# sd196821/QuadSim

Measured on AMD Instinct MI355X. Metric: env-steps/sec at N parallel envs (1/2/4/8 GPU); per-step state L2 err vs NumPy ref, higher is better.
Workload: dtype f32

## Files before the change

### quadsim_amd/csrc/private_queue.hpp

```cpp
#pragma once

struct QsChainLane {
    hsa_queue_t *queue = nullptr;
    char *kernargs = nullptr;
    std::vector<uint64_t> slot_qidx;
    uint64_t issued = 0;
    int64_t tile0 = 0, tile_end = 0;
    hsa_signal_t done{};
    void *rev_ptr = nullptr;
    hsa_signal_t rev{};
    int64_t rev_value = 0;
    char *res_kernarg = nullptr;
    hsa_signal_t res_done{};
    bool res_launched = false;
    uint64_t res_prog = 0;
};

struct QsKernel {
    uint64_t object = 0;
    uint32_t kernarg_size = 0, group_size = 0, private_size = 0;
    unsigned block = 0;
};

struct QsChain {
// ... 7 lines not shown
    std::vector<char> image;
    uint64_t kernel_object = 0;
    int v_integ = -1, v_params = -1, v_rmode = -1, v_split = -1, v_prep = -1;
    uint32_t kernarg_size = 0, group_size = 0, private_size = 0;
    unsigned block = 0;
    size_t stride = 0, slots = 0;
    unsigned *d_owner = nullptr;
    unsigned *d_err = nullptr;
    volatile unsigned *h_err = nullptr;
    bool kernargs_on_device = false;
    bool dirty = false;
    bool hip_dirty = true;
    bool stream_ordered = false;
    void *fwd_ptr = nullptr;
    hsa_signal_t fwd{};
    uint64_t fwd_seq = 0;
    int dbg_shift = 0;
    bool pkt_unreleased = false;
    bool res_enabled = false;
    bool res_dbg_packets = false;
    bool res_open = false;
    bool res_fits = false;
    QsKernel res_kernel;
    int rv_integ = -1, rv_params = -1, rv_rmode = -1, rv_prep = -1;
    int64_t res_wave_cap = 0;
    unsigned long long *ring = nullptr;
    size_t ring_slots = 0;
    uint64_t res_issued = 1;
    uint64_t res_retired = 1;
    uint64_t res_seq0 = 0;
    uint64_t res_idle_ticks = 0;
    uint64_t res_dispatches = 0;
    unsigned long long *d_rseq = nullptr;
    unsigned *d_rcnt = nullptr;
    volatile unsigned long long *h_res = nullptr;
    unsigned long long *d_hres = nullptr;
};

namespace {

#define HSA_TRY(expr)                                                                                   \
    do {                                                                                                \
        hsa_status_t s_ = (expr);                                                                       \
        if (s_ != HSA_STATUS_SUCCESS) {                                                                 \
            const char *m_ = nullptr;                                                                   \
            hsa_status_string(s_, &m_);                                                                 \
            return fail(QS_ERR_HIP, "%s failed: %s", #expr, m_ ? m_ : "unknown HSA status");           \
        }                                                                                               \
// ... 107 lines not shown
}

void chain_close(QsEnv *e)
{
    QsChain *c = e->chain;
    if (!c) return;
    if (c->fwd.handle) hsa_signal_store_screlease(c->fwd, INT64_MAX);
    for (QsChainLane &L : c->lanes) {
        if (L.queue) hsa_queue_destroy(L.queue);
        if (L.kernargs) hsa_amd_memory_pool_free(L.kernargs);
        if (L.done.handle) hsa_signal_destroy(L.done);
        if (L.rev_ptr) (void)hipFree(L.rev_ptr);
        if (L.res_kernarg) hsa_amd_memory_pool_free(L.res_kernarg);
        if (L.res_done.handle) hsa_signal_destroy(L.res_done);
    }
    if (c->ring) hsa_amd_memory_pool_free(c->ring);
    if (c->d_rseq) (void)hipFree(c->d_rseq);
    if (c->d_rcnt) (void)hipFree(c->d_rcnt);
    if (c->h_res) (void)hipHostFree((void *)c->h_res);
    if (c->fwd_ptr) (void)hipFree(c->fwd_ptr);
    if (c->have_exe) hsa_executable_destroy(c->exe);
    if (c->have_reader) hsa_code_object_reader_destroy(c->reader);
    if (c->d_owner) (void)hipFree(c->d_owner);
    if (c->h_err) (void)hipHostFree((void *)c->h_err);
    delete c;
    e->chain = nullptr;
}

int chain_resolve_kernel(QsEnv *e)
{
    QsChain *c = e->chain;
    const int integ = e->cfg.integrator == QS_INTEG_FROZEN ? 0 : 1;
    const int rmode = e->init ? 3 : e->cfg.randomise;
    const int params = (rmode == 2 || e->per_env_params) ? 1 : 0;
    static const int forced = getenv("QS_SPLIT") ? atoi(getenv("QS_SPLIT")) : -1;
    const int split = (forced >= 0 ? forced != 0 : e->n <= kSplitMaxEnvs) ? 1 : 0;
    int64_t lane_tiles = 0;
    for (const QsChainLane &L : c->lanes) lane_tiles = std::max<int64_t>(lane_tiles, L.tile_end - L.tile0);
    if (c->lanes.empty()) lane_tiles = e->tiles;
    const int prep = split ? prep_for(rmode, lane_tiles) : 0;
    if (c->kernel_object && integ == c->v_integ && rmode == c->v_rmode && params == c->v_params && split == c->v_split && prep == c->v_prep) return QS_OK;
    char sym[160];
    if (split) snprintf(sym, sizeof sym, "_ZN12_GLOBAL__N_111k_env_splitILi%dELb%dELi%dELi%dEEEvNS_8StepArgsE.kd", integ, params, rmode, prep);
    else snprintf(sym, sizeof sym, "_ZN12_GLOBAL__N_15k_envILi%dELb%dELi%dEEEvNS_8StepArgsE.kd", integ, params, rmode);
    hsa_executable_symbol_t ks;
    uint64_t ko = 0;
// ... 28 lines not shown
{
    int can = 0;
    return hipDeviceGetAttribute(&can, hipDeviceAttributeCanUseStreamWaitValue, e->cfg.device) == hipSuccess && can != 0;
}

int chain_enable_stream_order(QsEnv *e)
{
    QsChain *c = e->chain;
    if (!c->fwd_ptr) {
        int r = chain_alloc_hip_signal(&c->fwd_ptr, &c->fwd, 0);
        if (r) return r;
        c->fwd_seq = 0;
    }
    for (QsChainLane &L : c->lanes) {
        if (L.rev_ptr) continue;
        int r = chain_alloc_hip_signal(&L.rev_ptr, &L.rev, kRevStart);
        if (r) return r;
        L.rev_value = kRevStart;
    }
    c->stream_ordered = true;
    return QS_OK;
}

int chain_open(QsEnv *e, int nq)
{
    if (e->cfg.kind == QS_KIND_HOVERING_V0) return fail(QS_ERR_INVALID, "qs_set_queue_mode: docking envs only");
    if (e->cfg.io_space != QS_IO_DEVICE) return fail(QS_ERR_INVALID, "qs_set_queue_mode: device buffers only");
    QsChain *c = new (std::nothrow) QsChain();
    if (!c) return fail(QS_ERR_NOMEM, "qs_set_queue_mode: out of host memory");
    e->chain = c;
    auto body = [&]() -> int {
        HSA_TRY(hsa_init());
        char bus[32] = "";
        AgentPick pick{0xffffffffu, 0, e->cfg.device, 0, {}, {}, false, false};
        unsigned dom = 0, b = 0, d = 0, f = 0;
        if (hipDeviceGetPCIBusId(bus, sizeof bus, e->cfg.device) == hipSuccess && sscanf(bus, "%x:%x:%x.%x", &dom, &b, &d, &f) == 4) {
            pick.want_bdf = (b << 8) | (d << 3) | f;
            pick.want_domain = dom;
        }
        HSA_TRY(hsa_iterate_agents(chain_agent_cb, &pick));
        if (!pick.have_gpu || !pick.have_cpu) return fail(QS_ERR_HIP, "qs_set_queue_mode: no HSA agent for device %d (%s)", e->cfg.device, bus);
        c->gpu = pick.gpu; c->cpu = pick.cpu;
        hsa_status_t ps = hsa_amd_agent_iterate_memory_pools(c->cpu, chain_kernarg_pool_cb, &c->kernarg_pool);
        if (ps != HSA_STATUS_INFO_BREAK) return fail(QS_ERR_HIP, "qs_set_queue_mode: no kernarg memory pool");
        int r = chain_read_code_object(c->image);
        if (r) return r;
// ... 23 lines not shown
            L.tile0 = cut[q]; L.tile_end = cut[q + 1];
            HSA_TRY(hsa_queue_create(c->gpu, 4096, HSA_QUEUE_TYPE_SINGLE, nullptr, nullptr, UINT32_MAX, UINT32_MAX, &L.queue));
            if (dp.found) {
                HSA_TRY(hsa_amd_memory_pool_allocate(dp.pool, c->stride * c->slots, 0, (void **)&L.kernargs));
                HSA_TRY(hsa_amd_agents_allow_access(1, &c->cpu, nullptr, L.kernargs));
            } else {
                HSA_TRY(hsa_amd_memory_pool_allocate(c->kernarg_pool, c->stride * c->slots, 0, (void **)&L.kernargs));
                HSA_TRY(hsa_amd_agents_allow_access(1, &c->gpu, nullptr, L.kernargs));
            }
            memset(L.kernargs, 0, c->stride * c->slots);
            L.slot_qidx.assign(c->slots, 0);
            HSA_TRY(hsa_signal_create(0, 0, nullptr, &L.done));
        }
        HIP_TRY(hipMalloc((void **)&c->d_owner, (size_t)e->tiles * sizeof(unsigned)));
        HIP_TRY(hipHostMalloc((void **)&c->h_err, 64, hipHostMallocMapped | hipHostMallocCoherent));
        *c->h_err = 0;
        HIP_TRY(hipHostGetDevicePointer((void **)&c->d_err, (void *)c->h_err, 0));
        const char *res = getenv("QS_RESIDENT");
        c->res_enabled = dp.found && !(res && res[0] == '0');
        if (c->res_enabled) {
            int cus = 0;
            HIP_TRY(hipDeviceGetAttribute(&cus, hipDeviceAttributeMultiprocessorCount, e->cfg.device));
            c->res_wave_cap = (int64_t)cus * 4 * 3;
            const char *idle = getenv("QS_RESIDENT_IDLE_US");
            c->res_idle_ticks = (uint64_t)(idle ? std::max(1, atoi(idle)) : kResIdleUs) * 100;
            c->ring_slots = kResRingSlots;
            HSA_TRY(hsa_amd_memory_pool_allocate(dp.pool, c->ring_slots * kResWords * 8, 0, (void **)&c->ring));
            HSA_TRY(hsa_amd_agents_allow_access(1, &c->cpu, nullptr, c->ring));
            memset(c->ring, 0, c->ring_slots * kResWords * 8);
            for (QsChainLane &L : c->lanes) {
                HSA_TRY(hsa_amd_memory_pool_allocate(dp.pool, kResKernargBytes, 0, (void **)&L.res_kernarg));
                HSA_TRY(hsa_amd_agents_allow_access(1, &c->cpu, nullptr, L.res_kernarg));
                memset(L.res_kernarg, 0, kResKernargBytes);
                HSA_TRY(hsa_signal_create(0, 0, nullptr, &L.res_done));
            }
            HIP_TRY(hipMalloc((void **)&c->d_rseq, (size_t)e->tiles * sizeof(unsigned long long)));
            HIP_TRY(hipMalloc((void **)&c->d_rcnt, c->lanes.size() * 32 * sizeof(unsigned)));
            HIP_TRY(hipHostMalloc((void **)&c->h_res, c->lanes.size() * 64, hipHostMallocMapped | hipHostMallocCoherent));
            memset((void *)c->h_res, 0, c->lanes.size() * 64);
            HIP_TRY(hipHostGetDevicePointer((void **)&c->d_hres, (void *)c->h_res, 0));
        }
        const char *ord = getenv("QS_CHAIN_ORDER");
        if (!(ord && ord[0] == 'h') && chain_can_stream_order(e)) {
            r = chain_enable_stream_order(e);
            if (r) return r;
        }
        return QS_OK;
    };
    int rc;
    try { rc = body(); }
    catch (...) { rc = fail(QS_ERR_NOMEM, "qs_set_queue_mode: out of host memory"); }
    if (rc != QS_OK) chain_close(e);
    return rc;
}

enum { PKT_STEP = 0, PKT_BARRIER = 1, PKT_WAIT_VALUE = 2, PKT_RESIDENT = 3 };
uint64_t chain_write_packet(QsChain *c, QsChainLane &L, int kind, const void *kernarg, unsigned grid, int acquire, int release,
                            hsa_signal_t completion, hsa_signal_t wait_sig = hsa_signal_t{0}, int64_t wait_value = 0)
{
    const uint64_t idx = hsa_queue_add_write_index_relaxed(L.queue, 1);
    while (idx - hsa_queue_load_read_index_scacquire(L.queue) >= L.queue->size) __builtin_ia32_pause();
    void *slot = (char *)L.queue->base_address + (idx & (L.queue->size - 1)) * 64;
    uint32_t word0;
// ... 22 lines not shown
        p->grid_size_x = grid; p->grid_size_y = 1; p->grid_size_z = 1;
        p->private_segment_size = res ? c->res_kernel.private_size : c->private_size;
        p->group_segment_size = res ? c->res_kernel.group_size : c->group_size;
        p->kernel_object = res ? c->res_kernel.object : c->kernel_object;
        p->kernarg_address = (void *)kernarg;
        p->reserved2 = 0;
        p->completion_signal = completion;
        word0 = (uint16_t)((HSA_PACKET_TYPE_KERNEL_DISPATCH << HSA_PACKET_HEADER_TYPE) | fences) |
                ((uint32_t)(1 << HSA_KERNEL_DISPATCH_PACKET_SETUP_DIMENSIONS) << 16);
    }
    __atomic_store_n((uint32_t *)slot, word0, __ATOMIC_RELEASE);
    hsa_signal_store_screlease(L.queue->doorbell_signal, (hsa_signal_value_t)idx);
    return idx;
}


double res_now()
{
    timespec ts;
    clock_gettime(CLOCK_MONOTONIC, &ts);
    return (double)ts.tv_sec + 1e-9 * (double)ts.tv_nsec;
}

int res_resolve_kernel(QsEnv *e)
{
    QsChain *c = e->chain;
    if (!c->v_split) { c->res_fits = false; return QS_OK; }
    if (c->res_kernel.object && c->v_integ == c->rv_integ && c->v_params == c->rv_params && c->v_rmode == c->rv_rmode && c->v_prep == c->rv_prep)
        return QS_OK;
    char sym[200];
    snprintf(sym, sizeof sym, "_ZN12_GLOBAL__N_114k_env_residentILi%dELb%dELi%dELi%dEEEvNS_8StepArgsENS_7ResArgsE.kd", c->v_integ,
             c->v_params, c->v_rmode, c->v_prep);
    hsa_executable_symbol_t ks;
    QsKernel k;
    HSA_TRY(hsa_executable_get_symbol_by_name(c->exe, sym, &c->gpu, &ks));
    HSA_TRY(hsa_executable_symbol_get_info(ks, HSA_EXECUTABLE_SYMBOL_INFO_KERNEL_OBJECT, &k.object));
    HSA_TRY(hsa_executable_symbol_get_info(ks, HSA_EXECUTABLE_SYMBOL_INFO_KERNEL_KERNARG_SEGMENT_SIZE, &k.kernarg_size));
    HSA_TRY(hsa_executable_symbol_get_info(ks, HSA_EXECUTABLE_SYMBOL_INFO_KERNEL_GROUP_SEGMENT_SIZE, &k.group_size));
    HSA_TRY(hsa_executable_symbol_get_info(ks, HSA_EXECUTABLE_SYMBOL_INFO_KERNEL_PRIVATE_SEGMENT_SIZE, &k.private_size));
    if (k.kernarg_size > kResKernargBytes) return fail(QS_ERR_HIP, "queue mode: kernel argument block of %s is %u B", sym, k.kernarg_size);
    const int waves = split_waves(c->v_rmode, c->v_prep);
    k.block = (unsigned)(waves * kTile);
    c->res_kernel = k;
    c->rv_integ = c->v_integ; c->rv_params = c->v_params; c->rv_rmode = c->v_rmode; c->rv_prep = c->v_prep;
    c->res_fits = k.private_size == 0 && e->tiles * waves <= c->res_wave_cap;
    return QS_OK;
}

bool res_running(const QsChainLane &L) { return L.res_launched && hsa_signal_load_relaxed(L.res_done) != 0; }

int res_launch(QsEnv *e, QsChainLane &L, uint64_t seq0, uint64_t stop_seq)
{
    QsChain *c = e->chain;
    const size_t q = (size_t)(&L - c->lanes.data());
    StepArgs A = make_args(e);
    A.tile0 = L.tile0; A.tile_end = L.tile_end;
    A.T = 1;
    ResArgs R{};
    R.ring = c->ring;
    R.rseq = c->d_rseq;
    R.wcnt = c->d_rcnt + q * 32;
    R.fin = R.wcnt + kResWinSlots;
    R.h_prog = c->d_hres + q * 8;
    R.h_fin = R.h_prog + 1;
    R.seq0 = seq0;
    R.base = c->res_seq0;
    R.stop_seq = stop_seq;
    R.slots_mask = c->ring_slots - 1;
    R.idle_ticks = c->res_idle_ticks;
    R.lane_tiles = (unsigned)(L.tile_end - L.tile0);
    const size_t roff = (sizeof(StepArgs) + alignof(ResArgs) - 1) / alignof(ResArgs) * alignof(ResArgs);
    memcpy(L.res_kernarg, &A, sizeof A);
    memcpy(L.res_kernarg + roff, &R, sizeof R);
    __builtin_ia32_sfence();
    (void)*(volatile uint32_t *)(L.res_kernarg + roff + sizeof R - sizeof(uint32_t));
    hsa_signal_store_relaxed(L.res_done, 1);
    chain_write_packet(c, L, PKT_RESIDENT, L.res_kernarg, (unsigned)((L.tile_end - L.tile0) * c->res_kernel.block),
                       HSA_FENCE_SCOPE_SYSTEM, HSA_FENCE_SCOPE_SYSTEM, L.res_done);
    L.res_launched = true;
    ++c->res_dispatches;
    return QS_OK;
}

void res_refresh(QsChain *c)
{
    uint64_t m = UINT64_MAX;
    for (size_t q = 0; q < c->lanes.size(); ++q) {
        QsChainLane &L = c->lanes[q];
        L.res_prog = std::max<uint64_t>(L.res_prog, c->h_res[q * 8]);
        m = std::min<uint64_t>(m, L.res_prog);
    }
    c->res_retired = std::max<uint64_t>(c->res_retired, m);
}

int res_write(QsEnv *e, uint64_t s, int cmd, const StepArgs *A)
{
    QsChain *c = e->chain;
    if (c->res_retired + c->ring_slots <= s) {
        const double t_end = res_now() + kResTimeoutS;
        for (;;) {
            res_refresh(c);
            if (c->res_retired + c->ring_slots > s) break;
            for (QsChainLane &L : c->lanes)
                if (L.res_launched && !res_running(L)) { int r = res_launch(e, L, 0, UINT64_MAX); if (r) return r; }
            if (res_now() > t_end)
                return fail(QS_ERR_HIP, "queue mode: the resident step kernel consumed no descriptor for %.0f s (descriptor %llu, all "
                            "consumed below %llu, first lane's progress %llu, %llu dispatches)", kResTimeoutS, (unsigned long long)s,
                            (unsigned long long)c->res_retired, (unsigned long long)c->h_res[0], (unsigned long long)c->res_dispatches);
            __builtin_ia32_pause();
        }
    }
    const unsigned long long p[7] = {
        A ? (unsigned long long)A->actions : 0, A ? (unsigned long long)A->obs : 0, A ? (unsigned long long)A->reward : 0,
        A ? (unsigned long long)A->done : 0, A ? (unsigned long long)A->flags : 0, A ? (unsigned long long)A->term_obs : 0,
        A ? (unsigned long long)A->term_state : 0};
    for (int i = 0; i < 7; ++i)
        if (p[i] & ~kResPtrMask) return fail(QS_ERR_INVALID, "queue mode: a buffer address above 2^48");
    const unsigned long long tag = (unsigned long long)(s & 0xffff) << 48;
    volatile unsigned long long *w = c->ring + (s & (c->ring_slots - 1)) * kResWords;
    for (int i = 0; i < 7; ++i) w[i] = p[i] | tag;
    w[7] = ((unsigned long long)cmd << 32) | (unsigned long long)(uint32_t)(s >> 16) | tag;
    __builtin_ia32_sfence();
    return QS_OK;
}

int res_finish(QsEnv *e)
{
    QsChain *c = e->chain;
    if (!c->res_open) return QS_OK;
    const uint64_t s = c->res_issued;
    int r = res_write(e, s, 1, nullptr);
    if (r) return r;
    c->res_issued = s + 1;
    const double t_end = res_now() + kResTimeoutS;
    for (;;) {
        bool all = true;
        for (size_t q = 0; q < c->lanes.size(); ++q) {
            QsChainLane &L = c->lanes[q];
            if (res_running(L)) { all = false; continue; }
            if (hsa_signal_load_scacquire(L.res_done) == 0 && c->h_res[q * 8 + 1] >= s + 1) continue;
            r = res_launch(e, L, 0, s + 1);
            if (r) return r;
            all = false;
        }
        if (all) break;
        if (res_now() > t_end)
            return fail(QS_ERR_HIP, "queue mode: the resident step kernel did not end within %.0f s of its EXIT descriptor", kResTimeoutS);
        __builtin_ia32_pause();
    }
    c->res_retired = s + 1;
    c->res_open = false;
    return QS_OK;
}

int res_step(QsEnv *e, const StepArgs &A)
{
    QsChain *c = e->chain;
    if (!c->res_open) {
        if (c->hip_dirty) HIP_TRY(hipMemsetAsync(c->d_owner, 0xff, (size_t)e->tiles * sizeof(unsigned), e->stream));
        HIP_TRY(hipMemsetAsync(c->d_rcnt, 0, c->lanes.size() * 32 * sizeof(unsigned), e->stream));
        HIP_TRY(hipStreamSynchronize(e->stream));
        c->hip_dirty = false;
        if (c->pkt_unreleased) {
            for (QsChainLane &L : c->lanes)
                chain_write_packet(c, L, PKT_BARRIER, nullptr, 0, HSA_FENCE_SCOPE_NONE, HSA_FENCE_SCOPE_SYSTEM, hsa_signal_t{0});
            c->pkt_unreleased = false;
        }
        c->res_seq0 = c->res_issued;
        for (QsChainLane &L : c->lanes) L.res_launched = false;
        c->res_open = true;
    }
    const uint64_t s = c->res_issued;
    int r = res_write(e, s, 0, &A);
    if (r) return r;
    c->res_issued = s + 1;
    for (QsChainLane &L : c->lanes)
        if (!L.res_launched) { r = res_launch(e, L, c->res_seq0, UINT64_MAX); if (r) return r; }
        else if (!res_running(L)) { r = res_launch(e, L, 0, UINT64_MAX); if (r) return r; }
    return QS_OK;
}

int chain_drain(QsEnv *e)
{
    QsChain *c = e->chain;
    if (!c) return QS_OK;
    int rr = res_finish(e);
    if (!c->dirty) return rr;
    for (QsChainLane &L : c->lanes) {
        hsa_signal_store_relaxed(L.done, 1);
        chain_write_packet(c, L, PKT_BARRIER, nullptr, 0, HSA_FENCE_SCOPE_NONE, HSA_FENCE_SCOPE_SYSTEM, L.done);
    }
    const double t_end = res_now() + kResTimeoutS;
    for (QsChainLane &L : c->lanes)
        while (hsa_signal_wait_scacquire(L.done, HSA_SIGNAL_CONDITION_LT, 1, 1000000, HSA_WAIT_STATE_ACTIVE) != 0)
            if (res_now() > t_end) return fail(QS_ERR_HIP, "queue mode: the private queue did not drain within %.0f s", kResTimeoutS);
    c->dirty = false;
// ... 56 lines not shown
            (void)*(volatile uint32_t *)(ka[nl - 1] + sizeof A - sizeof(uint32_t));
        }
        const bool last = t + 1 == T;
        for (size_t q = 0; q < nl; ++q) {
            QsChainLane &L = c->lanes[q];
            const int64_t tiles = L.tile_end - L.tile0;
            const unsigned grid = c->v_split ? (unsigned)(tiles * c->block)
                                                        : (unsigned)(((tiles + kBlock / kTile - 1) / (kBlock / kTile)) * kBlock);
            const bool sig = c->stream_ordered && last;
            L.slot_qidx[slot[q]] = chain_write_packet(c, L, PKT_STEP, ka[q], grid, HSA_FENCE_SCOPE_AGENT,
                                                      sig ? HSA_FENCE_SCOPE_AGENT : HSA_FENCE_SCOPE_NONE, sig ? L.rev : hsa_signal_t{0});
            ++L.issued;
            if (sig) --L.rev_value;
        }
    }
    c->dirty = true;
    c->pkt_unreleased = true;
    if (c->stream_ordered)
        for (QsChainLane &L : c->lanes)
            HIP_TRY(hipStreamWaitValue64(e->stream, L.rev_ptr, (uint64_t)L.rev_value, hipStreamWaitValueEq, ~0ull));
    return QS_OK;
}

int chain_step(QsEnv *e, const StepArgs &A)
{
    QsChain *c = e->chain;
    if (c->res_enabled && !c->stream_ordered && !c->dbg_shift && !c->res_dbg_packets && !*c->h_err) {
        int r = chain_resolve_kernel(e);
        if (r) return r;
        r = res_resolve_kernel(e);
        if (r) return r;
        if (c->res_fits) {
            return res_step(e, A);
        }
    }
    return chain_submit(e, &A, 1);
}

}
```

### quadsim_amd/csrc/quadsim_hip.hip

```cpp
#include <hip/hip_runtime.h>
#include <hsa/hsa.h>
#include <hsa/hsa_ext_amd.h>
#include <hsa/amd_hsa_signal.h>

#include <elf.h>
#include <fcntl.h>
#include <sys/mman.h>
#include <sys/stat.h>
#include <unistd.h>

#include <cstdarg>
#include <cstdio>
#include <cstdlib>
#include <cstring>
#include <dlfcn.h>
#include <algorithm>
#include <atomic>
#include <condition_variable>
#include <mutex>
#include <new>
#include <thread>
#include <vector>

#ifdef QS_DEBUG
// ... 212 lines not shown
    static const int forced = getenv("QS_SPLIT") ? atoi(getenv("QS_SPLIT")) : -1;
    const bool split = forced >= 0 ? forced != 0 : A.n <= kSplitMaxEnvs;
    const int64_t tiles = A.tile_end - A.tile0;
    if (split && prep_for(RMODE, tiles) == 2 && (RMODE == 1 || RMODE == 2))
        hipLaunchKernelGGL((k_env_split<INTEG, PARAMS, RMODE, (RMODE == 1 || RMODE == 2) ? 2 : 0>), dim3((unsigned)tiles), dim3(3 * kTile), 0, s, A);
    else if (split) hipLaunchKernelGGL((k_env_split<INTEG, PARAMS, RMODE, 0>), dim3((unsigned)tiles), dim3(2 * kTile), 0, s, A);
    else hipLaunchKernelGGL((k_env<INTEG, PARAMS, RMODE>), dim3((unsigned)((tiles + kBlock / kTile - 1) / (kBlock / kTile))), dim3(kBlock), 0, s, A);
}

#define QS_RES_KERNELS(I)                                                                                               \
    template __global__ void k_env_resident<I, false, 0, 0>(StepArgs, ResArgs);                                         \
    template __global__ void k_env_resident<I, true, 0, 0>(StepArgs, ResArgs);                                          \
    template __global__ void k_env_resident<I, false, 1, 0>(StepArgs, ResArgs);                                         \
    template __global__ void k_env_resident<I, true, 1, 0>(StepArgs, ResArgs);                                          \
    template __global__ void k_env_resident<I, false, 1, 2>(StepArgs, ResArgs);                                         \
    template __global__ void k_env_resident<I, true, 1, 2>(StepArgs, ResArgs);                                          \
    template __global__ void k_env_resident<I, true, 2, 0>(StepArgs, ResArgs);                                          \
    template __global__ void k_env_resident<I, true, 2, 2>(StepArgs, ResArgs);                                          \
    template __global__ void k_env_resident<I, false, 3, 0>(StepArgs, ResArgs);                                         \
    template __global__ void k_env_resident<I, true, 3, 0>(StepArgs, ResArgs);
QS_RES_KERNELS(0)
QS_RES_KERNELS(1)
#undef QS_RES_KERNELS

template <int INTEG>
void launch_integ(hipStream_t s, const StepArgs &A, bool params, int rmode)
{
    if (rmode == 3) { if (params) launch_one<INTEG, true, 3>(s, A); else launch_one<INTEG, false, 3>(s, A); }
    else if (rmode == 2) launch_one<INTEG, true, 2>(s, A);
    else if (rmode == 1) { if (params) launch_one<INTEG, true, 1>(s, A); else launch_one<INTEG, false, 1>(s, A); }
    else { if (params) launch_one<INTEG, true, 0>(s, A); else launch_one<INTEG, false, 0>(s, A); }
}

int launch_env_on(QsEnv *e, const StepArgs &A, hipStream_t s)
{
    if (e->cfg.kind == QS_KIND_HOVERING_V0) {
        const unsigned grid = (unsigned)((A.tile_end - A.tile0 + kBlock / kTile - 1) / (kBlock / kTile));
        const bool fr = e->cfg.integrator == QS_INTEG_FROZEN, pp = e->per_env_params;
        if (fr && !pp) hipLaunchKernelGGL((k_hover<0, false>), dim3(grid), dim3(kBlock), 0, s, A);
        else if (fr) hipLaunchKernelGGL((k_hover<0, true>), dim3(grid), dim3(kBlock), 0, s, A);
        else if (!pp) hipLaunchKernelGGL((k_hover<1, false>), dim3(grid), dim3(kBlock), 0, s, A);
        else hipLaunchKernelGGL((k_hover<1, true>), dim3(grid), dim3(kBlock), 0, s, A);
        HIP_TRY(hipGetLastError());
        return QS_OK;
    }
    const int rmode = e->init ? 3 : e->cfg.randomise;
// ... 279 lines not shown
    if (mask) memcpy(B.host(d_mask), mask, n);
    if (obs_out && mask) {
        memcpy(B.host(d_obs), obs_out, n * od * sizeof(float));
        if (!B.direct) HIP_TRY(hipMemcpyAsync(d_obs, B.host(d_obs), n * od * sizeof(float), hipMemcpyHostToDevice, e->stream));
    }
    if (mask && (r = B.push())) return r;
    r = do_reset(e, mask ? d_mask : nullptr, d_obs, 0);
    if (r) return r;
    if ((r = B.pull())) return r;
    if (obs_out) memcpy(obs_out, B.host(d_obs), n * od * sizeof(float));
    return QS_OK;
}

int qs_step_ex(QsEnv *e, const float *actions, float *obs, float *reward, uint8_t *done, uint8_t *flags, float *terminal_obs,
               float *terminal_state)
{
    Range rg_("qs_step_ex");
    CHECK_ENV_RAW(e);
    if (!actions || !obs || !reward || !done) return fail(QS_ERR_INVALID, "qs_step: actions, obs, reward and done are required");
    if (terminal_state && e->cfg.kind == QS_KIND_HOVERING_V0)
        return fail(QS_ERR_INVALID, "qs_step_ex: hovering-v0 has no terminal_state (its terminal observation IS the state)");
    if (e->chain) {
        if (e->groups_dirty) { int rj = groups_join(e); if (rj) return rj; HIP_TRY(hipStreamSynchronize(e->stream)); }
        StepArgs A = make_args(e);
        A.actions = actions; A.obs = obs; A.reward = reward; A.done = done; A.flags = flags; A.term_obs = terminal_obs;
        A.term_state = terminal_state;
        return chain_step(e, A);
    }
    if (!e->groups.empty()) { int rcj = main_stream_entry(e); if (rcj) return rcj; }
    const int64_t n = e->n;
    StepArgs A = make_args(e);
    int r;
    if (e->cfg.io_space == QS_IO_DEVICE) {
        A.actions = actions; A.obs = obs; A.reward = reward; A.done = done; A.flags = flags; A.term_obs = terminal_obs;
        A.term_state = terminal_state;
        r = launch_env(e, A);
        if (r) return r;
    } else {
        const int64_t od = e->obs_dim;
        const size_t need = (size_t)n * (4 * 4 + od * 4 + 4 + 1 + 1 + od * 4 + 26 * 4) + 4096;
        r = ensure_stage(e, need);
        if (r) return r;
        Bounce B(e, need);
        float *d_act = B.take<float>(n * 4);
        B.inputs_done();
        float *d_obs = B.take<float>(n * od), *d_rew = B.take<float>(n);
// ... 770 lines not shown
    HIP_TRY(hipMemset(e->chain->d_owner, 9, (size_t)e->tiles * sizeof(unsigned)));
    e->chain->hip_dirty = false;
    e->chain->res_dbg_packets = true;
    return QS_OK;
}

int qs_debug_set_reset_prep(int mode) { return prep_forced().exchange((mode == 0 || mode == 2) ? mode : -1); }

int qs_debug_chain_shift_once(QsEnv *e, int32_t shift)
{
    if (!e || !e->chain) return fail(QS_ERR_INVALID, "qs_debug_chain_shift_once: not in private-queue mode");
    e->chain->dbg_shift = shift;
    e->chain->res_dbg_packets = true;
    return QS_OK;
}

int qs_debug_chain_resident(QsEnv *e, uint64_t *dispatches)
{
    if (!e || !dispatches) return fail(QS_ERR_INVALID, "qs_debug_chain_resident: null argument");
    *dispatches = e->chain ? e->chain->res_dispatches : 0;
    return QS_OK;
}

int qs_get_queue_ordering(QsEnv *e, int32_t *ordering)
{
    if (!e || !ordering) return fail(QS_ERR_INVALID, "qs_get_queue_ordering: null argument");
    *ordering = (e->chain && e->chain->stream_ordered) ? QS_ORDER_STREAM : QS_ORDER_HOST;
    return QS_OK;
}

int qs_set_queue_ordering(QsEnv *e, int32_t ordering)
{
    CHECK_ENV(e);
    if (!e->chain) return fail(QS_ERR_INVALID, "qs_set_queue_ordering: qs_set_queue_mode first");
    if (ordering != QS_ORDER_HOST && ordering != QS_ORDER_STREAM) return fail(QS_ERR_INVALID, "qs_set_queue_ordering: unknown ordering %d", ordering);
    QsChain *c = e->chain;
    if (c->stream_ordered && c->fwd_seq) HIP_TRY(hipStreamSynchronize(e->stream));
    if (ordering == QS_ORDER_HOST) { c->stream_ordered = false; return QS_OK; }
    if (!chain_can_stream_order(e))
        return fail(QS_ERR_INVALID, "qs_set_queue_ordering: this device / HIP runtime has no stream memory operations (hipStreamWaitValue64)");
    return chain_enable_stream_order(e);
}

int qs_get_queue_mode(QsEnv *e, int32_t *mode)
{
    if (!e || !mode) return fail(QS_ERR_INVALID, "qs_get_queue_mode: null argument");
// ... 137 lines not shown
```

### quadsim_amd/csrc/step_kernels.hpp

```cpp
#pragma once

namespace {

#ifndef QS_BLOCK
#define QS_BLOCK 256
#endif
constexpr int kBlock = QS_BLOCK;
#ifndef QS_PREP_MAX_TILES
#define QS_PREP_MAX_TILES 1365
#endif
constexpr int64_t kPrepMaxTiles = QS_PREP_MAX_TILES;
#ifndef QS_SPLIT_MAX_ENVS
#define QS_SPLIT_MAX_ENVS 131072
#endif
constexpr int64_t kSplitMaxEnvs = QS_SPLIT_MAX_ENVS;

struct StepArgs {
    float *st;
    float *par;
    const float *actions;
    float *obs;
    float *reward;
    uint8_t *done;
    uint8_t *flags;
// ... 587 lines not shown
        }
        QS_STAMP_AT(6);
        QS_STAMP_FLUSH();
    }
    else if (kPrep) {
        int64_t t = 0;
#pragma clang loop unroll(disable)
        for (; cmd == RES_STEP; ++t) {
            const uint64_t k = k0 + (uint64_t)t;
            uint4 w0, w1 = make_uint4(0, 0, 0, 0);
            random_init_words<RMODE == 2>(A.rc, STREAM_AUTORESET, A.gid0 + (uint64_t)env, k + 1, w0, w1);
            __syncthreads();
            float ic[13], it_[13], robs[12];
            Par Pn;
            random_init_apply<RMODE == 2>(A.rc, w0, w1, ic, it_, Pn);
            rel_obs<true>(ic, it_, robs);
#pragma unroll
            for (int i = 0; i < 13; ++i) s_rst[i][lane] = ic[i];
#pragma unroll
            for (int i = 0; i < 12; ++i) s_rst[13 + i][lane] = robs[i];
            if (PARAMS && RMODE == 2) {
                s_rst[25][lane] = Pn.m; s_rst[26][lane] = Pn.Ixx; s_rst[27][lane] = Pn.Iyy; s_rst[28][lane] = Pn.Izz;
            }
            __syncthreads();
            cmd = s_cmd[(t + 1) & 1];
        }
    }
}

template <int INTEG, bool PARAMS, int RMODE, int PREP>
__global__ __launch_bounds__(3 * kTile) void k_env_split(StepArgs A)
{
    __shared__ float s_tgt[13][kTile];
    constexpr bool kPrep = PREP == 2 && (RMODE == 1 || RMODE == 2);
    __shared__ float s_rst[kPrep ? 29 : 1][kTile];
    __shared__ uint4 s_phx[kPrep ? 1 : 2][kPrep ? 1 : 2][kTile];
    __shared__ unsigned char s_done[kTile], s_limt[kTile];
    const int lane = threadIdx.x & (kTile - 1);
    const int role = threadIdx.x >> 6;
    const int64_t tile = launch_tile(A, blockIdx.x);
    const int64_t env = tile * kTile + lane;
    bool active = env < A.n;
    const int64_t io = env - A.io_env0;
    QS_ASSERT(tile < A.tile_end && (!active || (io >= 0 && io < A.io_n)));
    const unsigned owner_xcc = chain_owner_request(A, tile);
    const uint64_t k0 = step_counter_begin_vmem(A, tile);
// ... 1147 lines not shown
        Roctx x;
        const char *en = getenv("QS_ROCTX");
        if (en && atoi(en)) {
            void *h = dlopen("librocprofiler-sdk-roctx.so", RTLD_NOW | RTLD_GLOBAL);
            if (!h) h = dlopen("libroctx64.so", RTLD_NOW | RTLD_GLOBAL);
            if (h) {
                x.push = (int (*)(const char *))dlsym(h, "roctxRangePushA");
                x.pop = (int (*)())dlsym(h, "roctxRangePop");
                x.on = x.push && x.pop;
            }
        }
        return x;
    }();
    return r;
}
struct Range {
    bool on;
    explicit Range(const char *name) : on(roctx().on) { if (on) roctx().push(name); }
    ~Range() { if (on) roctx().pop(); }
};

struct DeviceGuard {
    int prev = -1;
    bool ok = true;
    explicit DeviceGuard(int dev)
    {
        if (hipGetDevice(&prev) != hipSuccess) prev = -1;
        if (prev != dev) ok = hipSetDevice(dev) == hipSuccess;
    }
    ~DeviceGuard()
    {
        if (prev >= 0) (void)hipSetDevice(prev);
    }
};

inline int64_t tiles_of(int64_t n) { return (n + kTile - 1) / kTile; }
inline unsigned grid_tiles(int64_t n) { return (unsigned)((tiles_of(n) + (kBlock / kTile) - 1) / (kBlock / kTile)); }
inline unsigned grid_flat(int64_t n) { return (unsigned)((n + kBlock - 1) / kBlock); }

}
```

Baseline: 26.26 billion.

## Precompute deterministic target trajectory table for resident kernel and add host fast path

Measured after the change: 26.83 billion (median of 6 runs). +2.2%, better.

```diff
diff --git a/quadsim_amd/csrc/private_queue.hpp b/quadsim_amd/csrc/private_queue.hpp
--- a/quadsim_amd/csrc/private_queue.hpp
+++ b/quadsim_amd/csrc/private_queue.hpp
@@ -53,8 +53,15 @@
     bool res_open = false;
     bool res_fits = false;
     QsKernel res_kernel;
-    int rv_integ = -1, rv_params = -1, rv_rmode = -1, rv_prep = -1;
+    int rv_integ = -1, rv_params = -1, rv_rmode = -1, rv_prep = -1, rv_tab = -1;
     int64_t res_wave_cap = 0;
+    int res_cus = 0;
+    bool tab_enabled = false;
+    bool res_tab = false;
+    float *d_tab = nullptr;
+    bool tab_valid = false;
+    int tv_integ = -1, tv_kind = -1;
+    float tv_dt = 0.0f, tv_par[4] = {0.0f, 0.0f, 0.0f, 0.0f};
     unsigned long long *ring = nullptr;
     size_t ring_slots = 0;
     uint64_t res_issued = 1;
@@ -208,6 +215,7 @@
     if (c->have_exe) hsa_executable_destroy(c->exe);
     if (c->have_reader) hsa_code_object_reader_destroy(c->reader);
     if (c->d_owner) (void)hipFree(c->d_owner);
+    if (c->d_tab) (void)hipFree(c->d_tab);
     if (c->h_err) (void)hipHostFree((void *)c->h_err);
     delete c;
     e->chain = nullptr;
@@ -282,6 +290,8 @@
     return QS_OK;
 }
 
+int tab_ensure(QsEnv *e);
+
 int chain_open(QsEnv *e, int nq)
 {
     if (e->cfg.kind == QS_KIND_HOVERING_V0) return fail(QS_ERR_INVALID, "qs_set_queue_mode: docking envs only");
@@ -351,6 +361,9 @@
             int cus = 0;
             HIP_TRY(hipDeviceGetAttribute(&cus, hipDeviceAttributeMultiprocessorCount, e->cfg.device));
             c->res_wave_cap = (int64_t)cus * 4 * 3;
+            c->res_cus = cus;
+            const char *tab = getenv("QS_TARGET_TABLE");
+            c->tab_enabled = !(tab && tab[0] == '0');
             const char *idle = getenv("QS_RESIDENT_IDLE_US");
             c->res_idle_ticks = (uint64_t)(idle ? std::max(1, atoi(idle)) : kResIdleUs) * 100;
             c->ring_slots = kResRingSlots;
@@ -368,6 +381,7 @@
             HIP_TRY(hipHostMalloc((void **)&c->h_res, c->lanes.size() * 64, hipHostMallocMapped | hipHostMallocCoherent));
             memset((void *)c->h_res, 0, c->lanes.size() * 64);
             HIP_TRY(hipHostGetDevicePointer((void **)&c->d_hres, (void *)c->h_res, 0));
+            if (c->tab_enabled) { r = tab_ensure(e); if (r) return r; }
         }
         const char *ord = getenv("QS_CHAIN_ORDER");
         if (!(ord && ord[0] == 'h') && chain_can_stream_order(e)) {
@@ -436,15 +450,53 @@
     return (double)ts.tv_sec + 1e-9 * (double)ts.tv_nsec;
 }
 
+int tab_ensure(QsEnv *e)
+{
+    QsChain *c = e->chain;
+    const int integ = e->cfg.integrator == QS_INTEG_FROZEN ? 0 : 1;
+    const float par[4] = {e->cfg.mass, e->cfg.inertia[0], e->cfg.inertia[1], e->cfg.inertia[2]};
+    if (c->tab_valid && c->tv_integ == integ && c->tv_kind == e->cfg.kind && c->tv_dt == e->cfg.dt && !memcmp(c->tv_par, par, sizeof par))
+        return QS_OK;
+    c->tab_valid = false;
+    if (!c->d_tab) HIP_TRY(hipMalloc((void **)&c->d_tab, (size_t)(kTabLast + 1) * (kTabRecWords + kTabSideWords) * sizeof(float)));
+    const StepArgs A = make_args(e);
+    float *rec = c->d_tab, *side = c->d_tab + (size_t)(kTabLast + 1) * kTabRecWords;
+    if (integ == 0) hipLaunchKernelGGL(k_target_table<0>, dim3(1), dim3(kTile), 0, e->stream, A, rec, side);
+    else hipLaunchKernelGGL(k_target_table<1>, dim3(1), dim3(kTile), 0, e->stream, A, rec, side);
+    HIP_TRY(hipGetLastError());
+    HIP_TRY(hipStreamSynchronize(e->stream));
+    c->tv_integ = integ; c->tv_kind = e->cfg.kind; c->tv_dt = e->cfg.dt;
+    memcpy(c->tv_par, par, sizeof par);
+    c->tab_valid = true;
+    return QS_OK;
+}
+
+int tab_blocks_per_cu(int integ, int rmode, int *blocks)
+{
+    const int block = tab_waves(rmode) * kTile;
+    if (integ == 0 && rmode == 0) HIP_TRY(hipOccupancyMaxActiveBlocksPerMultiprocessor(blocks, k_env_resident_tab<0, 0>, block, 0));
+    else if (integ == 0) HIP_TRY(hipOccupancyMaxActiveBlocksPerMultiprocessor(blocks, k_env_resident_tab<0, 1>, block, 0));
+    else if (rmode == 0) HIP_TRY(hipOccupancyMaxActiveBlocksPerMultiprocessor(blocks, k_env_resident_tab<1, 0>, block, 0));
+    else HIP_TRY(hipOccupancyMaxActiveBlocksPerMultiprocessor(blocks, k_env_resident_tab<1, 1>, block, 0));
+    return QS_OK;
+}
+
 int res_resolve_kernel(QsEnv *e)
 {
     QsChain *c = e->chain;
     if (!c->v_split) { c->res_fits = false; return QS_OK; }
-    if (c->res_kernel.object && c->v_integ == c->rv_integ && c->v_params == c->rv_params && c->v_rmode == c->rv_rmode && c->v_prep == c->rv_prep)
+    const int tab = (c->tab_enabled && !c->v_params && (c->v_rmode == 0 || c->v_rmode == 1)) ? 1 : 0;
+    if (c->res_kernel.object && c->v_integ == c->rv_integ && c->v_params == c->rv_params && c->v_rmode == c->rv_rmode &&
+        c->v_prep == c->rv_prep && tab == c->rv_tab)
         return QS_OK;
+    if (tab) { int r = tab_ensure(e); if (r) return r; }
     char sym[200];
-    snprintf(sym, sizeof sym, "_ZN12_GLOBAL__N_114k_env_residentILi%dELb%dELi%dELi%dEEEvNS_8StepArgsENS_7ResArgsE.kd", c->v_integ,
-             c->v_params, c->v_rmode, c->v_prep);
+    if (tab)
+        snprintf(sym, sizeof sym, "_ZN12_GLOBAL__N_118k_env_resident_tabILi%dELi%dEEEvNS_8StepArgsENS_7ResArgsENS_7TabArgsE.kd",
+                 c->v_integ, c->v_rmode);
+    else
+        snprintf(sym, sizeof sym, "_ZN12_GLOBAL__N_114k_env_residentILi%dELb%dELi%dELi%dEEEvNS_8StepArgsENS_7ResArgsE.kd", c->v_integ,
+                 c->v_params, c->v_rmode, c->v_prep);
     hsa_executable_symbol_t ks;
     QsKernel k;
     HSA_TRY(hsa_executable_get_symbol_by_name(c->exe, sym, &c->gpu, &ks));
@@ -453,11 +505,19 @@
     HSA_TRY(hsa_executable_symbol_get_info(ks, HSA_EXECUTABLE_SYMBOL_INFO_KERNEL_GROUP_SEGMENT_SIZE, &k.group_size));
     HSA_TRY(hsa_executable_symbol_get_info(ks, HSA_EXECUTABLE_SYMBOL_INFO_KERNEL_PRIVATE_SEGMENT_SIZE, &k.private_size));
     if (k.kernarg_size > kResKernargBytes) return fail(QS_ERR_HIP, "queue mode: kernel argument block of %s is %u B", sym, k.kernarg_size);
-    const int waves = split_waves(c->v_rmode, c->v_prep);
+    const int waves = tab ? tab_waves(c->v_rmode) : split_waves(c->v_rmode, c->v_prep);
     k.block = (unsigned)(waves * kTile);
+    int64_t cap_tiles = c->res_wave_cap / waves;
+    if (tab) {
+        int nb = 0;
+        int r = tab_blocks_per_cu(c->v_integ, c->v_rmode, &nb);
+        if (r) return r;
+        cap_tiles = (int64_t)c->res_cus * nb;
+    }
     c->res_kernel = k;
-    c->rv_integ = c->v_integ; c->rv_params = c->v_params; c->rv_rmode = c->v_rmode; c->rv_prep = c->v_prep;
-    c->res_fits = k.private_size == 0 && e->tiles * waves <= c->res_wave_cap;
+    c->res_tab = tab != 0;
+    c->rv_integ = c->v_integ; c->rv_params = c->v_params; c->rv_rmode = c->v_rmode; c->rv_prep = c->v_prep; c->rv_tab = tab;
+    c->res_fits = k.private_size == 0 && e->tiles <= cap_tiles;
     return QS_OK;
 }
 
@@ -484,10 +544,17 @@
     R.idle_ticks = c->res_idle_ticks;
     R.lane_tiles = (unsigned)(L.tile_end - L.tile0);
     const size_t roff = (sizeof(StepArgs) + alignof(ResArgs) - 1) / alignof(ResArgs) * alignof(ResArgs);
+    const size_t toff = (roff + sizeof(ResArgs) + alignof(TabArgs) - 1) / alignof(TabArgs) * alignof(TabArgs);
     memcpy(L.res_kernarg, &A, sizeof A);
     memcpy(L.res_kernarg + roff, &R, sizeof R);
+    size_t end = roff + sizeof R;
+    if (c->res_tab) {
+        const TabArgs T{c->d_tab, c->d_tab + (size_t)(kTabLast + 1) * kTabRecWords};
+        memcpy(L.res_kernarg + toff, &T, sizeof T);
+        end = toff + sizeof T;
+    }
     __builtin_ia32_sfence();
-    (void)*(volatile uint32_t *)(L.res_kernarg + roff + sizeof R - sizeof(uint32_t));
+    (void)*(volatile uint32_t *)(L.res_kernarg + end - sizeof(uint32_t));
     hsa_signal_store_relaxed(L.res_done, 1);
     chain_write_packet(c, L, PKT_RESIDENT, L.res_kernarg, (unsigned)((L.tile_end - L.tile0) * c->res_kernel.block),
                        HSA_FENCE_SCOPE_SYSTEM, HSA_FENCE_SCOPE_SYSTEM, L.res_done);
@@ -507,7 +574,7 @@
     c->res_retired = std::max<uint64_t>(c->res_retired, m);
 }
 
-int res_write(QsEnv *e, uint64_t s, int cmd, const StepArgs *A)
+int res_write(QsEnv *e, uint64_t s, int cmd, const unsigned long long *p)
 {
     QsChain *c = e->chain;
     if (c->res_retired + c->ring_slots <= s) {
@@ -524,10 +591,8 @@
             __builtin_ia32_pause();
         }
     }
-    const unsigned long long p[7] = {
-        A ? (unsigned long long)A->actions : 0, A ? (unsigned long long)A->obs : 0, A ? (unsigned long long)A->reward : 0,
-        A ? (unsigned long long)A->done : 0, A ? (unsigned long long)A->flags : 0, A ? (unsigned long long)A->term_obs : 0,
-        A ? (unsigned long long)A->term_state : 0};
+    static const unsigned long long none[7] = {0, 0, 0, 0, 0, 0, 0};
+    if (!p) p = none;
     for (int i = 0; i < 7; ++i)
         if (p[i] & ~kResPtrMask) return fail(QS_ERR_INVALID, "queue mode: a buffer address above 2^48");
     const unsigned long long tag = (unsigned long long)(s & 0xffff) << 48;
@@ -567,7 +632,7 @@
     return QS_OK;
 }
 
-int res_step(QsEnv *e, const StepArgs &A)
+int res_step(QsEnv *e, const unsigned long long *p)
 {
     QsChain *c = e->chain;
     if (!c->res_open) {
@@ -585,7 +650,7 @@
         c->res_open = true;
     }
     const uint64_t s = c->res_issued;
-    int r = res_write(e, s, 0, &A);
+    int r = res_write(e, s, 0, p);
     if (r) return r;
     c->res_issued = s + 1;
     for (QsChainLane &L : c->lanes)
@@ -688,6 +753,12 @@
     return QS_OK;
 }
 
+bool chain_res_continues(const QsEnv *e)
+{
+    const QsChain *c = e->chain;
+    return c->res_open && c->res_fits && !c->stream_ordered && !c->dbg_shift && !c->res_dbg_packets && !*c->h_err;
+}
+
 int chain_step(QsEnv *e, const StepArgs &A)
 {
     QsChain *c = e->chain;
@@ -697,7 +768,10 @@
         r = res_resolve_kernel(e);
         if (r) return r;
         if (c->res_fits) {
-            return res_step(e, A);
+            const unsigned long long p[7] = {(unsigned long long)A.actions, (unsigned long long)A.obs, (unsigned long long)A.reward,
+                                             (unsigned long long)A.done, (unsigned long long)A.flags, (unsigned long long)A.term_obs,
+                                             (unsigned long long)A.term_state};
+            return res_step(e, p);
         }
     }
     return chain_submit(e, &A, 1);
diff --git a/quadsim_amd/csrc/quadsim_hip.hip b/quadsim_amd/csrc/quadsim_hip.hip
--- a/quadsim_amd/csrc/quadsim_hip.hip
+++ b/quadsim_amd/csrc/quadsim_hip.hip
@@ -258,6 +258,10 @@
 QS_RES_KERNELS(0)
 QS_RES_KERNELS(1)
 #undef QS_RES_KERNELS
+template __global__ void k_env_resident_tab<0, 0>(StepArgs, ResArgs, TabArgs);
+template __global__ void k_env_resident_tab<0, 1>(StepArgs, ResArgs, TabArgs);
+template __global__ void k_env_resident_tab<1, 0>(StepArgs, ResArgs, TabArgs);
+template __global__ void k_env_resident_tab<1, 1>(StepArgs, ResArgs, TabArgs);
 
 template <int INTEG>
 void launch_integ(hipStream_t s, const StepArgs &A, bool params, int rmode)
@@ -583,6 +587,12 @@
         return fail(QS_ERR_INVALID, "qs_step_ex: hovering-v0 has no terminal_state (its terminal observation IS the state)");
     if (e->chain) {
         if (e->groups_dirty) { int rj = groups_join(e); if (rj) return rj; HIP_TRY(hipStreamSynchronize(e->stream)); }
+        if (chain_res_continues(e)) {
+            const unsigned long long p[7] = {(unsigned long long)actions, (unsigned long long)obs, (unsigned long long)reward,
+                                             (unsigned long long)done, (unsigned long long)flags, (unsigned long long)terminal_obs,
+                                             (unsigned long long)terminal_state};
+            return res_step(e, p);
+        }
         StepArgs A = make_args(e);
         A.actions = actions; A.obs = obs; A.reward = reward; A.done = done; A.flags = flags; A.term_obs = terminal_obs;
         A.term_state = terminal_state;
@@ -1399,6 +1409,40 @@
     return QS_OK;
 }
 
+int qs_debug_resident_kernel(QsEnv *e, int32_t *table, int32_t *waves, int32_t *fits)
+{
+    if (!e || !table || !waves || !fits) return fail(QS_ERR_INVALID, "qs_debug_resident_kernel: null argument");
+    if (!e->chain) return fail(QS_ERR_INVALID, "qs_debug_resident_kernel: not in private-queue mode");
+    DeviceGuard guard(e->cfg.device);
+    QsChain *c = e->chain;
+    *table = 0; *waves = 0; *fits = 0;
+    if (!c->res_enabled) return QS_OK;
+    int r = chain_resolve_kernel(e);
+    if (r) return r;
+    r = res_resolve_kernel(e);
+    if (r) return r;
+    *table = c->res_tab ? 1 : 0;
+    *waves = c->res_kernel.object ? (int32_t)(c->res_kernel.block / kTile) : 0;
+    *fits = c->res_fits ? 1 : 0;
+    return QS_OK;
+}
+
+int qs_debug_target_table(QsEnv *e, float *rec, float *side)
+{
+    if (!e || !rec || !side) return fail(QS_ERR_INVALID, "qs_debug_target_table: null argument");
+    if (!e->chain) return fail(QS_ERR_INVALID, "qs_debug_target_table: not in private-queue mode");
+    DeviceGuard guard(e->cfg.device);
+    int r = chain_drain(e);
+    if (r) return r;
+    r = tab_ensure(e);
+    if (r) return r;
+    const QsChain *c = e->chain;
+    HIP_TRY(hipMemcpy(rec, c->d_tab, (size_t)(kTabLast + 1) * kTabRecWords * sizeof(float), hipMemcpyDeviceToHost));
+    HIP_TRY(hipMemcpy(side, c->d_tab + (size_t)(kTabLast + 1) * kTabRecWords, (size_t)(kTabLast + 1) * kTabSideWords * sizeof(float),
+                      hipMemcpyDeviceToHost));
+    return QS_OK;
+}
+
 int qs_get_queue_ordering(QsEnv *e, int32_t *ordering)
 {
     if (!e || !ordering) return fail(QS_ERR_INVALID, "qs_get_queue_ordering: null argument");
diff --git a/quadsim_amd/csrc/step_kernels.hpp b/quadsim_amd/csrc/step_kernels.hpp
--- a/quadsim_amd/csrc/step_kernels.hpp
+++ b/quadsim_amd/csrc/step_kernels.hpp
@@ -633,6 +633,314 @@
             if (PARAMS && RMODE == 2) {
                 s_rst[25][lane] = Pn.m; s_rst[26][lane] = Pn.Ixx; s_rst[27][lane] = Pn.Iyy; s_rst[28][lane] = Pn.Izz;
             }
+            __syncthreads();
+            cmd = s_cmd[(t + 1) & 1];
+        }
+    }
+}
+
+constexpr int kTabLast = (int)kTMax;
+constexpr int kTabRecWords = 16, kTabSideWords = 8;
+
+struct TabArgs {
+    const float *rec;
+    const float *side;
+};
+
+__device__ __forceinline__ bool qd_same_controller(const float a[4], const float b[4])
+{
+    float sa, ca, sha, cha, sb, cb, shb, chb;
+    quat_yaw_trig(a, sa, ca, sha, cha);
+    quat_yaw_trig(b, sb, cb, shb, chb);
+    return __float_as_uint(sa) == __float_as_uint(sb) && __float_as_uint(ca) == __float_as_uint(cb) &&
+           __float_as_uint(sha) == __float_as_uint(shb) && __float_as_uint(cha) == __float_as_uint(chb);
+}
+
+template <int INTEG>
+__global__ __launch_bounds__(kTile) void k_target_table(StepArgs A, float *rec, float *side)
+{
+    const int lane = threadIdx.x;
+    const Par P = A.par_nom;
+    const float pdes[3] = {10.0f, -50.0f, 5.0f};
+    const float vdes[3] = {A.C.vdes_x, 0.0f, 0.0f};
+    const float dv[3] = {0.0f, 0.0f, 0.0f};
+    float ic[13], st[13], ut[4] = {0.0f, 0.0f, 0.0f, 0.0f};
+    float qd[4] = {1.0f, 0.0f, 0.0f, 0.0f};
+    const float q0[4] = {1.0f, 0.0f, 0.0f, 0.0f};
+    nominal_init(ic, st);
+    bool lim = false;
+#pragma clang loop unroll(disable)
+    for (int j = 0; j <= kTabLast; ++j) {
+        if (j > 0) {
+            float pre[13];
+#pragma unroll
+            for (int i = 0; i < 13; ++i) pre[i] = st[i];
+            lim = drone_advance<INTEG>(st, ut, P, A.C.dt);
+            float u_t[4];
+            target_control(A.C.kind, pdes, vdes, qd, 0.0f, pre, dv, P.m, u_t);
+            u_limit(u_t, P.m * kG, ut);
+        }
+        const bool rejoin = qd_same_controller(qd, q0);
+        if (lane == 0) {
+            float *r = rec + (int64_t)j * kTabRecWords, *s = side + (int64_t)j * kTabSideWords;
+#pragma unroll
+            for (int i = 0; i < 13; ++i) r[i] = st[i];
+            r[13] = lim ? 1.0f : 0.0f;
+            r[14] = rejoin ? 1.0f : 0.0f;
+            r[15] = 0.0f;
+#pragma unroll
+            for (int i = 0; i < 4; ++i) { s[i] = ut[i]; s[4 + i] = qd[i]; }
+        }
+    }
+}
+
+__device__ __forceinline__ void tab_row(const TabArgs &T, int j, float st[13], bool &lim, bool &rejoin)
+{
+    const float4 *r = reinterpret_cast<const float4 *>(T.rec + (int64_t)j * kTabRecWords);
+    const float4 r0 = r[0], r1 = r[1], r2 = r[2], r3 = r[3];
+    st[0] = r0.x; st[1] = r0.y; st[2] = r0.z; st[3] = r0.w;
+    st[4] = r1.x; st[5] = r1.y; st[6] = r1.z; st[7] = r1.w;
+    st[8] = r2.x; st[9] = r2.y; st[10] = r2.z; st[11] = r2.w;
+    st[12] = r3.x;
+    lim = r3.y != 0.0f;
+    rejoin = r3.z != 0.0f;
+}
+
+__device__ __forceinline__ void tab_state(const TabArgs &T, int row, int qrow, float st[13], float ut[4], float qd[4])
+{
+    bool l, r;
+    tab_row(T, row, st, l, r);
+    const float4 *s = reinterpret_cast<const float4 *>(T.side + (int64_t)row * kTabSideWords);
+    const float4 *q = reinterpret_cast<const float4 *>(T.side + (int64_t)qrow * kTabSideWords);
+    const float4 u = s[0], d = q[1];
+    ut[0] = u.x; ut[1] = u.y; ut[2] = u.z; ut[3] = u.w;
+    qd[0] = d.x; qd[1] = d.y; qd[2] = d.z; qd[3] = d.w;
+}
+
+constexpr int tab_waves(int rmode) { return rmode == 1 ? 2 : 1; }
+
+template <int INTEG, int RMODE>
+__global__ __launch_bounds__(2 * kTile) void k_env_resident_tab(StepArgs A, ResArgs R, TabArgs T)
+{
+    static_assert(RMODE == 0 || RMODE == 1, "nominal or rocRAND-chaser resets only");
+    constexpr bool kPrepWave = RMODE == 1;
+    __shared__ float s_rst[kPrepWave ? 2 : 1][kPrepWave ? 25 : 1][kTile];
+    __shared__ int s_cmd[2];
+    const int lane = threadIdx.x & (kTile - 1);
+    const int role = threadIdx.x >> 6;
+    const int64_t tile = launch_tile(A, blockIdx.x);
+    const int64_t env = tile * kTile + lane;
+    const bool active = env < A.n;
+    const int64_t io = env - A.io_env0;
+    QS_ASSERT(tile < A.tile_end && (!active || (io >= 0 && io < A.io_n)));
+    const uint64_t k0 = step_counter_begin_vmem(A, tile);
+    unsigned long long seq = 0;
+    int cmd = RES_STEP;
+    ResDesc D{};
+    if (role == 0) {
+        seq = R.seq0 ? R.seq0 : R.rseq[tile];
+        seq = ((unsigned long long)__builtin_amdgcn_readfirstlane((int)(unsigned)(seq >> 32)) << 32) |
+              (unsigned)__builtin_amdgcn_readfirstlane((int)(unsigned)seq);
+        cmd = seq >= R.stop_seq ? RES_SKIP : res_resolve(R, seq, lane, res_request(R, seq, lane), D);
+        if (cmd == RES_STEP) res_report_done(R, res_report(R, seq, tile, lane), seq, tile, lane);
+        if (kPrepWave && lane == 0) s_cmd[0] = cmd;
+    } else if (kPrepWave) {
+        uint4 w0, w1 = make_uint4(0, 0, 0, 0);
+        random_init_words<false>(A.rc, STREAM_AUTORESET, A.gid0 + (uint64_t)env, k0 + 1, w0, w1);
+        float ic[13], it_[13], robs[12];
+        Par Pn;
+        random_init_apply<false>(A.rc, w0, w1, ic, it_, Pn);
+        rel_obs<true>(ic, it_, robs);
+#pragma unroll
+        for (int i = 0; i < 13; ++i) s_rst[0][i][lane] = ic[i];
+#pragma unroll
+        for (int i = 0; i < 12; ++i) s_rst[0][13 + i][lane] = robs[i];
+    }
+    if (kPrepWave) {
+        __syncthreads();
+        cmd = s_cmd[0];
+    }
+    const float *b = A.st + tile * (int64_t)(kRecWords * kTile) + lane;
+    float *bw = A.st + tile * (int64_t)(kRecWords * kTile) + lane;
+    const Par P = A.par_nom;
+    if (role == 0) {
+        __builtin_amdgcn_s_setprio(3);
+        QS_PHASE_DECL;
+        float sc[13], uc[4], st[13], ut[4], qd[4];
+#pragma unroll
+        for (int i = 0; i < 13; ++i) sc[i] = b[(F_SC + i) * kTile];
+#pragma unroll
+        for (int i = 0; i < 4; ++i) uc[i] = b[(F_UC + i) * kTile];
+        float ls = b[F_LS * kTile], tt = b[F_T * kTile];
+#pragma unroll
+        for (int i = 0; i < 13; ++i) st[i] = b[(F_ST + i) * kTile];
+#pragma unroll
+        for (int i = 0; i < 4; ++i) ut[i] = b[(F_UT + i) * kTile];
+#pragma unroll
+        for (int i = 0; i < 4; ++i) qd[i] = b[(F_QD + i) * kTile];
+        float4 av_next = make_float4(0.0f, 0.0f, 0.0f, 0.0f);
+        if (cmd == RES_STEP && active) av_next = res_action(D.actions, io, A.io_n);
+        int row = 0, qrow = 0;
+        bool on = true;
+        if (active) {
+            on = tt >= 0.0f && tt <= kTMax;
+            row = on ? (int)tt : 0;
+            on = on && (float)row == tt;
+            float rs_[13], ru[4], rq[4];
+            tab_state(T, row, row, rs_, ru, rq);
+#pragma unroll
+            for (int i = 0; i < 13; ++i) on = on && __float_as_uint(rs_[i]) == __float_as_uint(st[i]);
+#pragma unroll
+            for (int i = 0; i < 4; ++i) on = on && __float_as_uint(ru[i]) == __float_as_uint(ut[i]);
+            on = on && qd_same_controller(qd, rq);
+        }
+        bool exact = true;
+        const float pdes[3] = {10.0f, -50.0f, 5.0f};
+        const float vdes[3] = {A.C.vdes_x, 0.0f, 0.0f};
+        const float dv[3] = {0.0f, 0.0f, 0.0f};
+        const float q0[4] = {1.0f, 0.0f, 0.0f, 0.0f};
+        QS_PHASE(0);
+        int64_t t = 0;
+#pragma clang loop unroll(disable)
+        for (; cmd == RES_STEP; ++t) {
+            const int64_t o = io;
+            const unsigned long long wn = res_request(R, seq + t + 1, lane);
+            const bool on_step = on && row < kTabLast;
+            const bool tab = __all(on_step);
+            if (!tab && !exact) {
+                tab_state(T, row, qrow, st, ut, qd);
+                exact = true;
+            }
+            const int j = row + 1;
+            float stn[13];
+            bool lim_t, rejoin;
+            tab_row(T, tab ? j : 0, stn, lim_t, rejoin);
+            tt += 1.0f;
+            const bool lim_c = drone_advance<INTEG>(sc, uc, P, A.C.dt);
+            float a[4];
+            ResDesc Dn{};
+            unsigned rep = ~0u;
+            const float4 av = av_next;
+            QS_PHASE(1);
+            const int cmdn = res_resolve(R, seq + t + 1, lane, wn, Dn);
+            if (cmdn == RES_STEP) {
+                if (active) av_next = res_action(Dn.actions, io, A.io_n);
+                rep = res_report(R, seq + t + 1, tile, lane);
+            }
+            if (kPrepWave && lane == 0) s_cmd[(t + 1) & 1] = cmdn;
+            QS_PHASE(2);
+            a[0] = av.x; a[1] = av.y; a[2] = av.z; a[3] = av.w;
+            float u_c[4];
+            chaser_command(a, P.m, u_c);
+            u_limit(u_c, P.m * kG, uc);
+            if (!tab) {
+                float pre[13];
+#pragma unroll
+                for (int i = 0; i < 13; ++i) pre[i] = st[i];
+                lim_t = drone_advance<INTEG>(st, ut, P, A.C.dt);
+                float u_t[4];
+                target_control(A.C.kind, pdes, vdes, qd, 0.0f, pre, dv, P.m, u_t);
+                u_limit(u_t, P.m * kG, ut);
+#pragma unroll
+                for (int i = 0; i < 13; ++i) stn[i] = st[i];
+            }
+            float obs[12], reward;
+            unsigned flags;
+            rel_obs(sc, stn, obs);
+            score_step(obs, a, sc[2], tt, ls, A.C, lim_c, lim_t, reward, flags);
+            const bool done = (flags & (FLAG_OVERLIMIT | FLAG_OVERTIME)) != 0;
+            const bool rs = done && A.auto_reset;
+            if (active && on_step) { row = j; qrow = j; }
+            on = on && on_step;
+            if (rs) {
+                if (D.term_obs && active) store_obs(D.term_obs, io, obs);
+                if (D.term_state && active) {
+                    float *ts = D.term_state + io * 26;
+#pragma unroll
+                    for (int i = 0; i < 13; ++i) { ts[i] = sc[i]; ts[13 + i] = stn[i]; }
+                }
+                float ic[13], it[13];
+                nominal_init(ic, it);
+                if (RMODE == 0) {
+#pragma unroll
+                    for (int i = 0; i < 12; ++i) obs[i] = A.nominal_obs[i];
+                } else {
+#pragma unroll
+                    for (int i = 0; i < 13; ++i) ic[i] = s_rst[t & 1][i][lane];
+#pragma unroll
+                    for (int i = 0; i < 12; ++i) obs[i] = s_rst[t & 1][13 + i][lane];
+                }
+#pragma unroll
+                for (int i = 0; i < 13; ++i) sc[i] = ic[i];
+#pragma unroll
+                for (int i = 0; i < 4; ++i) uc[i] = 0.0f;
+                ls = 0.0f;
+                tt = 0.0f;
+                if (!tab) {
+                    nominal_init(ic, it);
+#pragma unroll
+                    for (int i = 0; i < 13; ++i) st[i] = it[i];
+#pragma unroll
+                    for (int i = 0; i < 4; ++i) ut[i] = 0.0f;
+                    rejoin = qd_same_controller(qd, q0);
+                }
+                if (active) { row = 0; on = rejoin; }
+            }
+            exact = !tab;
+            QS_PHASE(3);
+            if (active) {
+                store_obs(D.obs, o, obs);
+                QS_SO(&D.reward[o], reward);
+                QS_SO(&D.done[o], (uint8_t)(done ? 1 : 0));
+                if (D.flags) QS_SO(&D.flags[o], (uint8_t)flags);
+            }
+            res_report_done(R, rep, seq + t + 1, tile, lane);
+            D = Dn;
+            cmd = cmdn;
+            QS_PHASE(4);
+            if (kPrepWave) __syncthreads();
+            QS_PHASE(5);
+        }
+        if (t > 0 && active) {
+            if (!exact) tab_state(T, row, qrow, st, ut, qd);
+#pragma unroll
+            for (int i = 0; i < 13; ++i) QS_ST(&bw[(F_SC + i) * kTile], sc[i]);
+#pragma unroll
+            for (int i = 0; i < 4; ++i) QS_ST(&bw[(F_UC + i) * kTile], uc[i]);
+            QS_ST(&bw[F_LS * kTile], ls);
+            QS_ST(&bw[F_T * kTile], tt);
+#pragma unroll
+            for (int i = 0; i < 13; ++i) QS_ST(&bw[(F_ST + i) * kTile], st[i]);
+#pragma unroll
+            for (int i = 0; i < 4; ++i) QS_ST(&bw[(F_UT + i) * kTile], ut[i]);
+#pragma unroll
+            for (int i = 0; i < 4; ++i) QS_ST(&bw[(F_QD + i) * kTile], qd[i]);
+        }
+        if (cmd != RES_SKIP && lane == 0) {
+            if (t > 0) A.ctr[tile] = k0 + (uint64_t)t;
+            R.rseq[tile] = seq + (unsigned long long)t + (cmd == RES_EXIT ? 1 : 0);
+            if (cmd == RES_EXIT) {
+                const unsigned old = __hip_atomic_fetch_add(R.fin, 1u, __ATOMIC_RELAXED, __HIP_MEMORY_SCOPE_AGENT);
+                if (old + 1 == R.lane_tiles)
+                    __hip_atomic_store(R.h_fin, seq + (unsigned long long)t + 1, __ATOMIC_RELAXED, __HIP_MEMORY_SCOPE_SYSTEM);
+            }
+        }
+        QS_PHASE(0);
+        QS_PHASE_FLUSH(0);
+    } else if (kPrepWave) {
+        int64_t t = 0;
+#pragma clang loop unroll(disable)
+        for (; cmd == RES_STEP; ++t) {
+            uint4 w0, w1 = make_uint4(0, 0, 0, 0);
+            random_init_words<false>(A.rc, STREAM_AUTORESET, A.gid0 + (uint64_t)env, k0 + (uint64_t)t + 2, w0, w1);
+            float ic[13], it_[13], robs[12];
+            Par Pn;
+            random_init_apply<false>(A.rc, w0, w1, ic, it_, Pn);
+            rel_obs<true>(ic, it_, robs);
+#pragma unroll
+            for (int i = 0; i < 13; ++i) s_rst[(t + 1) & 1][i][lane] = ic[i];
+#pragma unroll
+            for (int i = 0; i < 12; ++i) s_rst[(t + 1) & 1][13 + i][lane] = robs[i];
             __syncthreads();
             cmd = s_cmd[(t + 1) & 1];
         }
@@ -1826,15 +2134,15 @@
 
 struct DeviceGuard {
     int prev = -1;
-    bool ok = true;
+    bool ok = true, switched = false;
     explicit DeviceGuard(int dev)
     {
         if (hipGetDevice(&prev) != hipSuccess) prev = -1;
-        if (prev != dev) ok = hipSetDevice(dev) == hipSuccess;
+        if (prev != dev) { ok = hipSetDevice(dev) == hipSuccess; switched = true; }
     }
     ~DeviceGuard()
     {
-        if (prev >= 0) (void)hipSetDevice(prev);
+        if (switched && prev >= 0) (void)hipSetDevice(prev);
     }
 };
 
```
